# ZhangXiaze/DeepPointMap

Measured on AMD Instinct MI355X. Metric: LiDAR frames/s (encode+match+register), 65 536 pts/frame, higher is better.
Workload: dtype f32 (attention scores K Q^T and P V, Linear / Conv1d (+ LayerNorm) layers with K <= 2048 as exact three-way bf16 splits: 6 bf16 products per fp32 product, fp32 accumulate -- fp32 accuracy, bf16 matrix pipe; all else fp32); 1 GPU; synthetic 64x65536-pt scans per GPU: Encoder.forward + consecutive-frame registration_forward (256x256) + information matrix per frame; points_per_frame=65536, parallelism=frame-sharded x1, one RCCL gather of descriptors+edges per step, weights=procedural (deeppointmap_amd/weights.py), allocator_reserve_gib=16, geometry_waits_for_caller_stream=True

## Files before the change

### deeppointmap_amd/_lib.py

```python
from __future__ import annotations

import ctypes
import os

import torch
from ctypes import c_char_p, c_double, c_int, c_longlong, c_size_t, c_void_p

_HERE = os.path.dirname(os.path.abspath(__file__))
LIB_PATH = os.environ.get("DPM_LIB") or os.path.join(_HERE, "libdpm_hip.so")
VERSION_EXPERIMENT = 0x40000000

P, I, D, LL = c_void_p, c_int, c_double, c_longlong

SIGNATURES = {
    "dpm_version": (I, []),
    "dpm_error_string": (c_char_p, [I]),
    "dpm_prepare_points": (I, [P, P, I, I, I, P, P, P]),
    "dpm_to_channel_first": (I, [P, I, I, I, P, P]),
    "dpm_to_channel_first_ld": (I, [P, I, I, I, P, I, P]),
    "dpm_emit_descriptors": (I, [P, P, P, I, I, I, D, P, P, P, P, P]),
    "dpm_nested_levels": (I, [P, P, I, I, I, P, P, P, P, P]),
    "dpm_gather_frames": (I, [P, LL, I, I, I, P, I, P, P]),
    "dpm_fps_workspace_bytes": (c_size_t, [I, I, I]),
    "dpm_fps": (I, [P, P, I, I, I, P, P, P, P, P]),
    "dpm_fps_ex": (I, [P, P, I, I, I, P, P, P, P, I, P]),
    "dpm_fps_start": (I, [P, P, P, I, I, I, P, P, P, P, P]),
    "dpm_knn_workspace_bytes": (c_size_t, [I, I]),
    "dpm_knn_hybrid": (I, [P, P, P, I, I, I, I, D, P, P, P]),
    "dpm_knn_hybrid_reuse": (I, [P, P, P, I, I, I, I, D, P, P, P, P, P]),
    "dpm_knn_build_grid": (I, [P, P, I, I, D, P, P]),
    "dpm_knn_hybrid_prebuilt": (I, [P, P, P, I, I, I, I, D, P, P, P]),
    "dpm_ball_query": (I, [P, P, P, I, I, I, I, D, P, P]),
    "dpm_voxel_sampler_bounds": (I, [P, P, I, I, I, D, D, P, P]),
    "dpm_voxel_sampler_workspace_bytes": (c_size_t, [I, I, LL]),
    "dpm_voxel_sampler_select": (I, [P, P, I, I, I, D, D, P, LL, I, P, I, P, P, P]),
    "dpm_posegraph_optimize": (I, [P, I, P, P, P, P, I, I, P, P, P]),
    "dpm_host_topk_replay": (I, [P, I, I, I, P]),
    "dpm_host_sort_replay": (I, [P, I, I, P]),
    "dpm_group_mlp_max": (I, [P, P, P, P, P, P, P, P, I, I, I, I, I, I, D, P, P]),
    "dpm_group_mlp_max_generic": (I, [P, P, P, P, P, P, P, P, I, I, I, I, I, I, D, P, P]),
    "dpm_group_mlp_max_from_xyz": (I, [P, P, P, P, P, P, P, P, P, I, I, I, I, I, I, D, P, P]),
    "dpm_group_gather_ln_max": (I, [P, P, P, P, P, I, P, P, I, I, I, I, I, D, P, P]),
    "dpm_group_gather_ln_max_folded": (I, [P, P, P, P, I, P, P, I, I, I, I, I, D, P, P]),
    "dpm_group_affine_ln_max": (I, [P, P, P, P, P, P, I, P, P, I, I, I, I, I, D, P, P]),
    "dpm_group_gather_ln_max_centred": (I, [P, P, P, P, I, P, P, I, I, I, I, I, D, P, P]),
    "dpm_group_affine_ln_max_centred": (I, [P, P, P, P, P, P, I, P, P, I, I, I, I, I, D, P, P]),
    "dpm_linear": (I, [P, I, P, I, P, P, I, P, I, I, I, I, I, P]),
    "dpm_linear_batched": (I, [P, I, LL, P, I, LL, P, P, I, LL, P, I, LL, I, I, I, I, I, P]),
    "dpm_split_bf16x3": (I, [P, LL, P, P]),
    "dpm_linear_bf16x3": (I, [P, I, P, I, LL, P, P, I, P, I, I, I, I, I, P]),
    "dpm_linear_bf16x3_rank3": (I, [P, I, P, I, LL, P, P, I, P, I, I, I, I, I, P, P, I, D, P]),
    "dpm_linear_layernorm_bf16x3": (I, [P, I, P, I, LL, P, P, P, P, P, P, I, I, I, I, I, P]),
    "dpm_pwconv_pair_bf16x3": (I, [P, I, P, LL, P, P, P, P, LL, P, P, P, P, P, I, I, I, P]),
    "dpm_layernorm": (I, [P, I, P, P, P, P, P, I, I, I, I, P]),
    "dpm_linear_layernorm": (I, [P, I, P, I, P, P, P, P, P, P, I, I, I, I, I, P]),
    "dpm_three_interp_cat": (I, [P, P, P, P, P, I, I, I, I, I, P, P]),
    "dpm_posemb": (I, [P, I, P, I, I, I, P, P]),
    "dpm_attention": (I, [P, I, LL, P, I, LL, P, I, LL, P, I, LL, I, I, I, I, I, P]),
    "dpm_attention_shifted": (I, [P, I, LL, P, I, LL, P, I, LL, P, I, LL, I, I, I, I, I, I, P]),
    "dpm_attention_masked": (I, [P, I, LL, P, I, LL, P, I, LL, P, I, LL, I, I, I, I, I, I, P, P]),
    "dpm_attention_indexed": (I, [P, I, LL, P, I, LL, P, I, LL, P, I, LL, I, I, I, I, I, I, P, P]),
    "dpm_attention_split_workspace_bytes": (c_size_t, [I, I, I, I, I]),
# ... 56 lines not shown
    "dpm_offset_pairs_segment_sum": (I, [P, I, P, P, LL, I, P, P]),
    "dpm_group_train_forward": (I, [P, P, P, P, P, I, P, P, I, I, I, I, I, D, P, P, P]),
    "dpm_group_train_workspace_bytes": (c_size_t, [I, I, I, I, I]),
    "dpm_group_train_backward": (I, [P, P, P, P, P, I, P, I, I, I, I, I, D, P, P, P, P, P, P, P, P]),
    "dpm_loop_pool_workspace_bytes": (c_size_t, [I, I, I]),
    "dpm_loop_pool_forward": (I, [P, I, P, P, I, I, I, P, P, P]),
    "dpm_loop_pool_backward": (I, [P, I, P, P, P, I, I, I, P, P, P, P]),
    "dpm_loop_bce_forward": (I, [P, P, I, P, P, P, P]),
    "dpm_dense_train_workspace_bytes": (c_size_t, [LL, I, I]),
    "dpm_dense_train_forward": (I, [P, I, P, I, P, P, P, P, P, LL, I, I, I, P, P, P, P]),
    "dpm_dense_train_backward_rows": (I, [P, P, P, P, P, LL, I, I, P, P, P, P, P, P]),
    "dpm_dense_train_backward_gemm": (I, [P, P, I, P, I, LL, I, I, P, P, P, P, P]),
    "dpm_map_poses": (I, [P, P, P, P, P, I, I, I, P, P, P]),
    "dpm_map_assemble_fwd": (I, [P, P, P, P, P, I, I, I, I, I, D, P, P, P, P, P, P, P]),
    "dpm_map_assemble_bwd": (I, [P, P, I, I, I, I, I, P, P]),
    "dpm_optim_chunk": (I, []),
    "dpm_optim_step": (I, [I, P, P, I, D, D, D, D, D, D, D, D, I, I, P]),
    "dpm_flat_pack": (I, [P, P, I, P, LL, P]),
    "dpm_flat_unpack": (I, [P, P, I, P, LL, P]),
    "dpm_optim_step_synced": (I, [I, P, P, I, D, D, D, D, D, D, D, D, I, I, P, I, LL, D, P]),
    "dpm_lidar_cull": (I, [P, P, I, P, P, I, D, I, P, P, P, P]),
    "dpm_lidar_cast": (I, [P, P, P, I, I, P, I, I, D, D, P, P, P, P]),
    "dpm_lidar_cull_sweep": (I, [P, P, I, P, P, P, I, I, D, I, P, P, P, P, P]),
    "dpm_lidar_cast_sweep": (I, [P, P, P, I, I, P, I, I, P, I, D, D, P, P, P, P]),
    "dpm_lidar_emit": (I, [P, P, P, P, I, I, P, P, D, P, P, I, P, P, P, P, P, P]),
    "dpm_scene_distance": (I, [P, I, P, I, D, I, D, D, D, P, P, P]),
    "dpm_cloud_nn_workspace_bytes": (c_size_t, [I, I]),
    "dpm_cloud_nn": (I, [P, I, P, I, D, D, D, D, P, P, P, P]),
    "dpm_distance_stats_workspace_bytes": (c_size_t, [I, I, I]),
    "dpm_distance_stats": (I, [P, I, P, P, I, I, P, I, D, P, P, P]),
}


class DpmError(RuntimeError):
    pass


_lib = None


def load() -> ctypes.CDLL:
    global _lib
    if _lib is None:
        if not os.path.exists(LIB_PATH):
            raise DpmError(
                f"{LIB_PATH} not found: the HIP extension is not built. "
                "Run `python deeppointmap_amd/csrc/build.py` (there is no CPU fallback)."
            )
        lib = ctypes.CDLL(LIB_PATH)
        for name, (res, args) in SIGNATURES.items():
            fn = getattr(lib, name)
            fn.restype, fn.argtypes = res, args
        if lib.dpm_version() & VERSION_EXPERIMENT:
            import sys
            print(f"deeppointmap_amd: {LIB_PATH} is an EXPERIMENTAL build (-DDPM_EXPERIMENT): its kernels read DPM_* "
                  "measurement switches from the environment, some of which skip work -- not for results", file=sys.stderr)
        _lib = lib
    return _lib


def experimental() -> bool:
    return bool(load().dpm_version() & VERSION_EXPERIMENT)


def check(status: int, what: str) -> None:
    if status == 0:
# ... 6 lines not shown
```

### deeppointmap_amd/csrc/knn.hip

```cpp
#include "block_scan.h"
#include "filter_dc.h"
#include "topk_emulate.h"
#include <type_traits>

namespace {

constexpr int CPW = 4;
constexpr int WPB = 4;
constexpr int CAP = 512;
constexpr int KMAX = 64;
constexpr int TMPN = 128;
constexpr int GDIM = 128;
constexpr int GRID_MIN_N = 1024;
constexpr int KNN_TODO_MARK = -2;

using LdsF = __attribute__((address_space(3))) volatile float *;
using LdsI = __attribute__((address_space(3))) volatile int *;

__device__ __forceinline__ void wave_mem_sync() {
    __builtin_amdgcn_fence(__ATOMIC_SEQ_CST, "wavefront");
    __builtin_amdgcn_wave_barrier();
}

__device__ __forceinline__ float sq3(float x, float y, float z) { return (x * x + y * y) + z * z; }

__device__ __forceinline__ float exp_dist(float cx, float cy, float cz, float caa, float x, float y, float z,
                                          float bb) {
    return ((-2.f * fmaf(cz, z, fmaf(cy, y, cx * x))) + caa) + bb;
}

__device__ __forceinline__ int fkey(float d) {
    const int u = __float_as_int(d);
    return u >= 0 ? u : (u ^ 0x7fffffff);
}

// ... 276 lines not shown
    } else {
        for (int p = lane; p < c.cnt; p += 64) ti[p] = ci[p];
        wave_mem_sync();
    }
    const bool heap_regime = (long long)K * 64 <= (long long)N;
    bool exact_here = c.tie && len >= K && (heap_regime || tie_count || nth_row);
    if (exact_here && tie_count) {
        int slot = 0;
        if (lane == 0) slot = atomicAdd(tie_count, 1);
        slot = __shfl(slot, 0, 64);
        if (slot < TIE_CAP) {
            if (lane == 0) tie_rows[slot] = row;
            exact_here = false;
        }
    }
    if (exact_here && !heap_regime && !nth_row) exact_here = false;
    if (exact_here) {
        wave_mem_sync();
        if (heap_regime) heap_select_exact(pts, len, K, c.x, c.y, c.z, c.aa, cd, ci, td);
        else nth_select_exact(pts, len, N, K, c.x, c.y, c.z, c.aa, nth_row, cd, ci);
        emit_heap_result(cd, ci, K, r2, out);
    } else {
        int outv = (lane < k) ? ti[lane] : first;
        const unsigned long long hm = __ballot(lane < k && outv == first);
        const int L = hm ? __builtin_ctzll(hm) : 0;
        const int v0 = __shfl(outv, 0, 64);
        if (lane == L) outv = v0;
        if (lane == 0) outv = first;
        if (lane < K) out[lane] = outv;
    }
    wave_mem_sync();
}

__global__ __launch_bounds__(WPB * 64) void knn_hybrid_kernel(const float *__restrict__ points_all,
                                                              const int32_t *__restrict__ lengths,
                                                              const float *__restrict__ centers_all, int N,
                                                              int S, int K, float r2,
                                                              int32_t *__restrict__ idx_all,
                                                              const int32_t *__restrict__ reuse_idx,
                                                              const int32_t *__restrict__ center_src, int nth_rows) {
    extern __shared__ VI s_nth[];
    __shared__ float s_d[WPB][CPW][CAP];
    __shared__ int s_i[WPB][CPW][CAP];
    __shared__ float s_td[WPB][TMPN];
    __shared__ int s_ti[WPB][TMPN];
    const int b = blockIdx.y, w = threadIdx.x >> 6, lane = threadIdx.x & 63;
    const int s0 = (blockIdx.x * WPB + w) * CPW;
    if (s0 >= S) return;
    if (reuse_idx) {
        bool all = true;
        for (int j = 0; j < CPW && s0 + j < S; ++j) all &= center_src[(size_t)b * S + s0 + j] >= 0;
        if (all) {
            for (int j = 0; j < CPW && s0 + j < S; ++j) {
                const int src = center_src[(size_t)b * S + s0 + j];
                if (lane < K) idx_all[((size_t)b * S + s0 + j) * K + lane] = reuse_idx[((size_t)b * N + src) * K + lane];
            }
            return;
        }
    }
    const float *pts = points_all + (size_t)b * N * 3;
    const float *ctr = centers_all + (size_t)b * S * 3;
    const int len = min(max(lengths[b], 0), N);
    Ctr c[CPW];
#pragma unroll
    for (int j = 0; j < CPW; ++j) ctr_init(c[j], ctr + 3 * (size_t)min(s0 + j, S - 1), r2);
    for (int base = 0; base < len; base += 64) {
        const int i = base + lane;
        const bool ok = i < len;
        float x = 0.f, y = 0.f, z = 0.f;
        if (ok) x = pts[3 * i], y = pts[3 * i + 1], z = pts[3 * i + 2];
        const float bb = sq3(x, y, z);
#pragma unroll
        for (int j = 0; j < CPW; ++j) offer(c[j], ok, x, y, z, bb, i, K, (LdsF)s_d[w][j], (LdsI)s_i[w][j], (LdsF)s_td[w], (LdsI)s_ti[w]);
    }
#pragma unroll
    for (int j = 0; j < CPW; ++j) {
        if (s0 + j >= S) break;
        finish(c[j], pts, len, N, K, r2, (LdsF)s_d[w][j], (LdsI)s_i[w][j], (LdsF)s_td[w], (LdsI)s_ti[w],
               idx_all + ((size_t)b * S + (s0 + j)) * K, nullptr, nullptr, 0,
               nth_rows ? (VI *)((char *)s_nth + (size_t)w * N * (sizeof(VI) + 4)) : nullptr);
    }
}

struct KnnGrid {
    float lox, loy, inv_cs;
    int g;
    float err2;
    int H;
    int h;
    int pad;
};

constexpr float GRID_RHO_POINTS = 128.f;
constexpr float GRID_PI = 3.14159265f;

__global__ __launch_bounds__(1024) void knn_grid_build_kernel(const float *__restrict__ points_all,
                                                              const int32_t *__restrict__ lengths, int N,
                                                              float cs_min, float r2_margin, KnnGrid *__restrict__ hdr_all,
                                                              int *__restrict__ start_all,
                                                              float4 *__restrict__ sorted_all,
                                                              int *__restrict__ tie_count) {
    if (blockIdx.x == 0 && threadIdx.x == 0) tie_count[0] = 0, tie_count[1] = 0;
    __shared__ int s_hist[GDIM * GDIM];
    __shared__ float s_red[4][16];
    __shared__ float s_m2[16];
    __shared__ int s_wsum[16];
    const int b = blockIdx.x, t = threadIdx.x, lane = t & 63, w = t >> 6;
    const float *pts = points_all + (size_t)b * N * 3;
    const int len = min(max(lengths[b], 0), N);
    float lox = __builtin_inff(), loy = lox, hix = -lox, hiy = -lox, m2 = 0.f;
    constexpr int UB = 8;
    auto for_points = [&](auto &&fn) {
        for (int i0 = t; i0 < len; i0 += 1024 * UB) {
            float xs[UB], ys[UB], zs[UB];
// ... 881 lines not shown
}

extern "C" int dpm_knn_hybrid_reuse(const float *points, const int32_t *lengths, const float *centers, int B, int N,
                                    int S, int K, double radius, int32_t *idx, void *workspace,
                                    const int32_t *reuse_idx, const int32_t *center_src, dpm_stream_t stream) {
    DPM_CHECK_ARG(points && lengths && centers && idx);
    DPM_CHECK_ARG((reuse_idx == nullptr) == (center_src == nullptr));
    DPM_CHECK_ARG(B >= 1 && N >= 1 && S >= 1 && K >= 1 && radius > 0.0);
    if (K > KMAX) return DPM_EUNSUPPORTED;
    hipStream_t st = (hipStream_t)stream;
    const float r2 = (float)(radius * radius);
    if (N >= GRID_MIN_N && workspace) {
        const KnnWs w = carve(workspace, B, N);
        launch_grid_build(points, lengths, B, N, radius, w, st);
        return launch_grid_search(points, lengths, centers, B, N, S, K, r2, idx, w, reuse_idx, center_src, st);
    }
    int nth_rows = (long long)K * 64 > (long long)N;
    size_t dyn = nth_rows ? (sizeof(VI) + 4) * (size_t)WPB * N : 0;
    if (dyn) {
        static size_t static_lds = 0;
        if (!static_lds) {
            hipFuncAttributes fa;
            static_lds = hipFuncGetAttributes(&fa, (const void *)knn_hybrid_kernel) == hipSuccess ? fa.sharedSizeBytes : 72 * 1024;
        }
        if (static_lds + dyn > 160 * 1024) nth_rows = 0, dyn = 0;
        else if (dyn > 32 * 1024)
            (void)hipFuncSetAttribute((const void *)knn_hybrid_kernel, hipFuncAttributeMaxDynamicSharedMemorySize, (int)dyn);
    }
    hipLaunchKernelGGL(knn_hybrid_kernel, dim3(dpm_cdiv(S, WPB * CPW), B), dim3(WPB * 64), dyn, st, points, lengths, centers, N, S,
                       K, r2, idx, reuse_idx, center_src, nth_rows);
    return dpm_launch_status();
}

extern "C" int dpm_knn_build_grid(const float *points, const int32_t *lengths, int B, int N, double radius,
                                  void *workspace, dpm_stream_t stream) {
    DPM_CHECK_ARG(points && lengths && workspace && B >= 1 && N >= GRID_MIN_N && radius > 0.0);
    launch_grid_build(points, lengths, B, N, radius, carve(workspace, B, N), (hipStream_t)stream);
    return dpm_launch_status();
}

extern "C" int dpm_knn_hybrid_prebuilt(const float *points, const int32_t *lengths, const float *centers, int B, int N,
                                       int S, int K, double radius, int32_t *idx, void *workspace,
                                       dpm_stream_t stream) {
    DPM_CHECK_ARG(points && lengths && centers && idx && workspace);
    DPM_CHECK_ARG(B >= 1 && N >= GRID_MIN_N && S >= 1 && K >= 1 && radius > 0.0);
    if (K > KMAX) return DPM_EUNSUPPORTED;
    return launch_grid_search(points, lengths, centers, B, N, S, K, (float)(radius * radius), idx, carve(workspace, B, N),
                              nullptr, nullptr, (hipStream_t)stream);
}

extern "C" int dpm_knn_hybrid(const float *points, const int32_t *lengths, const float *centers, int B, int N,
                              int S, int K, double radius, int32_t *idx, void *workspace, dpm_stream_t stream) {
    return dpm_knn_hybrid_reuse(points, lengths, centers, B, N, S, K, radius, idx, workspace, nullptr, nullptr, stream);
}

extern "C" size_t dpm_knn_self_workspace_bytes(int N) { return dpm_knn_workspace_bytes(1, N > GRID_MIN_N ? N : GRID_MIN_N); }

extern "C" int dpm_knn_self(const float *xyz, int N, int K, double cell, int32_t *idx, float *dist2, float *mean_dist,
                            void *workspace, dpm_stream_t stream) {
    DPM_CHECK_ARG(xyz && workspace && N >= 1 && K >= 1 && cell > 0.0 && (idx || dist2 || mean_dist));
    if (K + 1 > KMAX) return DPM_EUNSUPPORTED;
    hipStream_t st = (hipStream_t)stream;
    uintptr_t p = ((uintptr_t)workspace + 255) & ~(uintptr_t)255;
    KnnGrid *hdr = (KnnGrid *)p;
    p = (p + sizeof(KnnGrid) + 255) & ~(uintptr_t)255;
    int *start = (int *)p;
// ... 119 lines not shown
```

### deeppointmap_amd/encoder.py

```python
from __future__ import annotations

from typing import List, Optional

import torch
from torch.utils.checkpoint import checkpoint

from . import ops
from .params import ParamTree, encoder_shapes


class Encoder(ParamTree):
    def __init__(self, args):
        super().__init__(encoder_shapes(args))
        self.args = args
        self.encoder_cfg = args.encoder
        self.in_channel = self.encoder_cfg.in_channel
        self.out_channel = self.encoder_cfg.out_channel
        self.downsample_layers = len(self.encoder_cfg.npoint)
        self.upsample_layers = self.encoder_cfg.upsample_layers
        for s in self.encoder_cfg.sample:
            if s["type"] not in ("fps", "fps-t3d", "voxel"):
                raise ValueError(f"{dict(s)} is not a supported sampling way, please use 'fps' or 'voxel'")
            if s["type"] == "voxel" and not ("size" in s and "range" in s):
                raise ValueError("a voxel sampler needs 'size' and 'range'")
        self.all_fps = all(s["type"] != "voxel" for s in self.encoder_cfg.sample)
        self.nested_fps = self.all_fps and all(b <= a for a, b in zip(self.encoder_cfg.npoint, self.encoder_cfg.npoint[1:]))
        self.presample_neighbours = False
        self.presample_neighbours_from = None
        self._price_tail = 0
        self.train_checkpoint_rows = 1 << 20
        self._was_trained = False
        self.eval()

    @property
    def device(self) -> torch.device:
        return self.p("point_mlp0.weight").device

    def _mlp_ln(self, x: torch.Tensor, conv: str, ln: str, act: int, post: Optional[torch.Tensor] = None):
        return ops.linear_layernorm(x, self.p(conv + ".weight"), self.p(conv + ".bias"), self.p(ln + ".weight"),
                                    self.p(ln + ".bias"), act=act, post=post)
# ... 60 lines not shown
                    if key not in answered and pts_i.shape[1] >= ops.GRID_MIN_N:
                        grids[("la", i, key)] = ops.knn_grid(pts_i, len_i, radii[j])
                    answered.add(key)
            out["grids"] = grids
            if n_levels == len(self.encoder_cfg.npoint):
                if self.presample_neighbours:
                    out["knn"] = self._neighbour_queries(out)
                elif self.presample_neighbours_from is not None:
                    out["knn"] = self._neighbour_queries(out, first_level=int(self.presample_neighbours_from))
        return out

    def _neighbour_queries(self, samp: dict, first_level: int = 0) -> dict:
        enc, grids, knn = self.encoder_cfg, samp.get("grids", {}), {}
        xyz, lengths, self_q = samp["xyz"], samp["lengths"], {}
        for i in range(len(enc.npoint)):
            radii, ks = enc.radius_list[i], enc.nsample_list[i]
            fidx, new_xyz, new_len = samp[f"fidx{i}"], samp[f"xyz{i}"], samp[f"len{i}"]
            if i < first_level:
                xyz, lengths, self_q = new_xyz, new_len, {}
                continue
            prev = self_q.get((float(radii[0]), int(ks[0])))
            knn[("sa", i)] = ops.knn_hybrid(xyz, lengths, new_xyz, ks[0], radii[0], reuse_idx=prev,
                                            center_src=fidx if prev is not None else None,
                                            grid=grids.get(("sa", i)) if prev is None else None)
            self_q = {}
            for j in range(1, len(radii)):
                key = (float(radii[j]), int(ks[j]))
                if key not in self_q:
                    self_q[key] = ops.knn_hybrid(new_xyz, new_len, new_xyz, ks[j], radii[j], grid=grids.get(("la", i, key)))
                knn[("la", i, key)] = self_q[key]
            xyz, lengths = new_xyz, new_len
        return knn

    @torch.no_grad()
    def forward(self, points: torch.Tensor, points_padding: torch.Tensor, trace: Optional[dict] = None,
                presampled: Optional[dict] = None, descriptor_scale: float = 0.0, spare_frames: int = 0,
                stop_level: Optional[int] = None, resume: Optional[dict] = None) -> List[torch.Tensor]:
        dev = self._require_gpu()
        if self.training and self.train_stage != "loop_detection":
            for name, given in (("presampled", presampled is not None), ("descriptor_scale", descriptor_scale != 0.0),
                                ("spare_frames", spare_frames != 0), ("stop_level", stop_level is not None),
                                ("resume", resume is not None)):
                if given:
                    raise ValueError(f"Encoder.forward: `{name}` belongs to the inference pipeline and is not available in "
                                     f".train() mode (call .eval() first)")
            return self._forward_train(points, points_padding, trace)
        enc = self.encoder_cfg
        if resume is not None:
            samp = resume["samp"]
        else:
            samp = presampled if presampled is not None else self.presample(points, points_padding)
        with torch.cuda.device(dev):
            pts, xyz, lengths = samp["pts"], samp["xyz"], samp["lengths"]
            w0 = self.p("point_mlp0.weight")
            fuse0 = (self.in_channel == 3 and w0.shape[0] % 4 == 0 and 2 * w0.shape[0] in (32, 64, 128)
                     and enc.nsample_list[0][0] in (16, 32))
            if resume is not None or fuse0:
                fea = None
            elif self.in_channel == 3:
                fea = ops.linear(xyz, w0, self.p("point_mlp0.bias"))
            else:
                fea = ops.linear(pts[:, :self.in_channel].transpose(1, 2).contiguous(), w0, self.p("point_mlp0.bias"))
            levels = [(xyz, fea, lengths)] if resume is None else resume["levels"]
            self_q = {} if resume is None else resume["self_q"]
            for i, npoint in enumerate(enc.npoint):
                if resume is not None and i < resume["next"]:
                    continue
                if stop_level is not None and i >= stop_level:
                    return dict(samp=samp, levels=levels, self_q=self_q, next=i)
                xyz, fea, lengths = levels[-1]
                radii, ks = enc.radius_list[i], enc.nsample_list[i]
                pre = f"downsampler.{i}"
                if f"fidx{i}" in samp:
                    fidx, new_xyz, new_len = samp[f"fidx{i}"], samp[f"xyz{i}"], samp[f"len{i}"]
                else:
                    fidx, new_xyz, new_len = self._sample_level(i, xyz, lengths)
                for _rep in range(1 + (self._price_tail if i >= 3 else 0)):
                    prev = self_q.get((float(radii[0]), int(ks[0])))
                    grids, knn = samp.get("grids", {}), samp.get("knn", {})
                    gidx = knn.get(("sa", i))
                    if gidx is None:
                        gidx = ops.knn_hybrid(xyz, lengths, new_xyz, ks[0], radii[0], reuse_idx=prev,
                                              center_src=fidx if prev is not None else None,
                                              grid=grids.get(("sa", i)) if prev is None else None)
                    self_q = {}
                    if fea is None:
                        m = pre + ".sa.mlp"
                        new_fea = ops.group_mlp_max_from_xyz(xyz, w0, self.p("point_mlp0.bias"), new_xyz, gidx,
                                                             self.p(m + ".0.weight"), self.p(m + ".0.bias"),
                                                             self.p(m + ".1.ln.weight"), self.p(m + ".1.ln.bias"), radii[0])
                    else:
                        new_fea = self._group(pre + ".sa.mlp", radii[0], xyz, fea, new_xyz, gidx)
                    if trace is not None:
                        trace[pre + ".fps.idx"], trace[pre + ".fps.new"] = fidx, new_xyz
                        trace[pre + ".sa.idx"], trace[pre + ".sa.out"] = gidx, new_fea
                    for j in range(1, len(radii)):
                        q = f"{pre}.irm.{j - 1}"
                        key = (float(radii[j]), int(ks[j]))
                        if key not in self_q:
                            self_q[key] = knn[("la", i, key)] if ("la", i, key) in knn else ops.knn_hybrid(
                                new_xyz, new_len, new_xyz, ks[j], radii[j], grid=grids.get(("la", i, key)))
                        lidx = self_q[key]
                        t = self._group(q + ".la.mlp", radii[j], new_xyz, new_fea, new_xyz, lidx)
                        pair = ops.pwconv_pair(t, self.p(q + ".pw_conv.0.weight"), self.p(q + ".pw_conv.0.bias"),
                                               self.p(q + ".pw_conv.1.ln.weight"), self.p(q + ".pw_conv.1.ln.bias"),
                                               self.p(q + ".pw_conv.3.weight"), self.p(q + ".pw_conv.3.bias"),
                                               self.p(q + ".pw_conv.4.ln.weight"), self.p(q + ".pw_conv.4.ln.bias"), post=new_fea)
                        if pair is not None:
                            new_fea = pair
                        else:
                            u = self._mlp_ln(t, q + ".pw_conv.0", q + ".pw_conv.1.ln", ops.ACT_RELU)
                            new_fea = self._mlp_ln(u, q + ".pw_conv.3", q + ".pw_conv.4.ln", ops.ACT_RELU, post=new_fea)
# ... 119 lines not shown
```

### deeppointmap_amd/knobs.py

```python
from __future__ import annotations

import os

FPS_ALGO = None
FUSED_LN = True
GEMM_BF16X3 = True
BF16X3_MAX_K = 2048
GEMM_LN_BF16X3 = True
BF16X3_LN_MIN_K = 128
FUSED_LN_SMALL_ROWS = 0
FOLD_GATHER = True
FOLD_MIN_RADIUS = 0.2
CENTRED_GATHER = True
FUSED_PWCONV = True
FUSED_MATCH = True
KV_PLANES = True
DEDUP_FRAMES = True

_ENV = {"DPM_FOLD_MIN_RADIUS": ("FOLD_MIN_RADIUS", float), "DPM_KV_PLANES": ("KV_PLANES", lambda v: v != "0"), "DPM_CENTRED_GATHER": ("CENTRED_GATHER", lambda v: v != "0"), "DPM_FPS_ALGO": ("FPS_ALGO", int), "DPM_NO_FUSED_LN": ("FUSED_LN", lambda v: v != "1"),
        "DPM_DEDUP_FRAMES": ("DEDUP_FRAMES", lambda v: v != "0"), "DPM_GEMM_BF16X3": ("GEMM_BF16X3", lambda v: v == "1"), "DPM_BF16X3_MAX_K": ("BF16X3_MAX_K", int), "DPM_BF16X3_LN_MIN_K": ("BF16X3_LN_MIN_K", int), "DPM_FUSED_LN_SMALL_ROWS": ("FUSED_LN_SMALL_ROWS", int), "DPM_GEMM_LN_BF16X3": ("GEMM_LN_BF16X3", lambda v: v == "1"),
        "DPM_FUSED_MATCH": ("FUSED_MATCH", lambda v: v != "0"), "DPM_FUSED_PWCONV": ("FUSED_PWCONV", lambda v: v != "0"), "DPM_FOLD_GATHER": ("FOLD_GATHER", lambda v: v != "0")}


def env_knobs() -> dict:
    return {k: v for k, v in sorted(os.environ.items()) if k.startswith("DPM_")}


def apply_env() -> dict:
    g = globals()
    for var, (name, conv) in _ENV.items():
        if var in os.environ:
            g[name] = conv(os.environ[var])
    return env_knobs()
```

### deeppointmap_amd/ops.py

```python
from __future__ import annotations

from typing import Optional, Tuple

import ctypes
import threading
import weakref

import torch

from . import _lib, knobs

ACT_NONE, ACT_RELU, ACT_SIGMOID = 0, 1, 2


def _ptr(t: Optional[torch.Tensor]):
    return None if t is None else t.data_ptr()


def _stream(t: torch.Tensor):
    return torch.cuda.current_stream(t.device).cuda_stream


def _chk(t: torch.Tensor, dtype, name: str):
    if not t.is_cuda:
# ... 112 lines not shown
    lib = _lib.load()
    ws = torch.empty(lib.dpm_knn_workspace_bytes(B, N), device=points.device, dtype=torch.uint8)
    _lib.check(lib.dpm_knn_build_grid(_ptr(points), _ptr(lengths), B, N, float(radius), _ptr(ws), _stream(points)),
               "dpm_knn_build_grid")
    return ws


def knn_hybrid(points: torch.Tensor, lengths: torch.Tensor, centers: torch.Tensor, K: int,
               radius: float, brute: bool = False, reuse_idx: Optional[torch.Tensor] = None,
               center_src: Optional[torch.Tensor] = None, grid: Optional[torch.Tensor] = None) -> torch.Tensor:
    _chk(points, torch.float32, "points")
    _chk(centers, torch.float32, "centers")
    _chk(lengths, torch.int32, "lengths")
    B, N, _ = points.shape
    S = centers.shape[1]
    idx = torch.empty(B, S, K, device=points.device, dtype=torch.int32)
    lib = _lib.load()
    if grid is not None:
        if brute or reuse_idx is not None or grid.numel() != lib.dpm_knn_workspace_bytes(B, N):
            raise ValueError("grid= goes with a plain grid search of the (B, N) it was built for")
        _lib.check(lib.dpm_knn_hybrid_prebuilt(_ptr(points), _ptr(lengths), _ptr(centers), B, N, S, K, float(radius),
                                               _ptr(idx), _ptr(grid), _stream(points)), "dpm_knn_hybrid_prebuilt")
        return idx
    nbytes = 0 if brute else lib.dpm_knn_workspace_bytes(B, N)
    ws = torch.empty(nbytes, device=points.device, dtype=torch.uint8) if nbytes else None
    if reuse_idx is not None:
        _chk(reuse_idx, torch.int32, "reuse_idx"), _chk(center_src, torch.int32, "center_src")
        if tuple(reuse_idx.shape) != (B, N, K) or tuple(center_src.shape) != (B, S):
            raise ValueError("reuse_idx must be (B,N,K) and center_src (B,S)")
    _lib.check(lib.dpm_knn_hybrid_reuse(_ptr(points), _ptr(lengths), _ptr(centers), B, N, S, K, float(radius),
                                        _ptr(idx), _ptr(ws), _ptr(reuse_idx), _ptr(center_src), _stream(points)),
               "dpm_knn_hybrid")
    return idx


def ball_query(points: torch.Tensor, lengths: torch.Tensor, centers: torch.Tensor, K: int, radius: float) -> torch.Tensor:
    _chk(points, torch.float32, "points"), _chk(centers, torch.float32, "centers"), _chk(lengths, torch.int32, "lengths")
    B, N, _ = points.shape
    S = centers.shape[1]
    idx = torch.empty(B, S, K, device=points.device, dtype=torch.int32)
    _lib.check(_lib.load().dpm_ball_query(_ptr(points), _ptr(lengths), _ptr(centers), B, N, S, K, float(radius),
                                          _ptr(idx), _stream(points)), "dpm_ball_query")
    return idx


VOXEL_SAMPLER_MAX_CELLS = 1 << 28
VOXEL_SAMPLER_MAX_WORKSPACE = 64 << 30


def voxel_sample(points: torch.Tensor, padding: torch.Tensor, K: Optional[int], voxel_size: float = 0.3,
                 sample_range: float = 1.0):
    _chk(points, torch.float32, "points")
    if padding.dtype != torch.bool or tuple(padding.shape) != tuple(points.shape[:2]):
        raise ValueError("points_padding must be a (B,N) bool tensor")
    B, N, D = points.shape
    if K is None and B != 1:
        raise ValueError("K=None takes one frame (utils.py:200)")
    lib, dev, st = _lib.load(), points.device, _stream(points)
    pad = padding.contiguous().view(torch.uint8)
    hdr = torch.empty(B, 8, device=dev, dtype=torch.float32)
    _lib.check(lib.dpm_voxel_sampler_bounds(_ptr(points), _ptr(pad), B, N, D, float(voxel_size), float(sample_range),
                                            _ptr(hdr), st), "dpm_voxel_sampler_bounds")
    dims = hdr[:, 3:6].double().cpu()
    if not bool(torch.isfinite(dims).all()):
        raise ValueError("voxel sampler: the frame's bounding box is not finite")
    cells = int(dims.prod(1).max().item())
# ... 1682 lines not shown
```

### include/dpm_hip.h

```cpp
#ifndef DPM_HIP_H
#define DPM_HIP_H

#include <stddef.h>
#include <stdint.h>

#ifdef __cplusplus
extern "C" {
#endif

typedef void *dpm_stream_t;

#define DPM_OK 0
#define DPM_EINVAL (-1)
#define DPM_EUNSUPPORTED (-2)

#define DPM_ACT_NONE 0
#define DPM_ACT_RELU 1
#define DPM_ACT_SIGMOID 2

#define DPM_VERSION_EXPERIMENT 0x40000000
int dpm_version(void);
const char *dpm_error_string(int status);

int dpm_prepare_points(const float *points_cf, const uint8_t *padding, int B, int C, int N,
                       float *xyz, int32_t *lengths, dpm_stream_t stream);

int dpm_to_channel_first(const float *x, int B, int R, int C, float *out, dpm_stream_t stream);
int dpm_to_channel_first_ld(const float *x, int B, int R, int C, float *out, int ldo, dpm_stream_t stream);

int dpm_emit_descriptors(const float *xyz, const float *fea, const int32_t *lengths, int B, int S, int C,
                         double coor_scale, float *coor, float *feat, uint8_t *padding, float *desc, dpm_stream_t stream);

int dpm_nested_levels(const float *xyz0, const int32_t *len0, int B, int K0, int n_levels, const int32_t *npoint,
                      float *xyz_out, int32_t *idx_out, int32_t *len_out, dpm_stream_t stream);

int dpm_gather_frames(const float *src, long long frame_stride, int rows, int ld, int cols, const int32_t *index, int n,
                      float *out, dpm_stream_t stream);

size_t dpm_fps_workspace_bytes(int B, int N, int K);
int dpm_fps(const float *xyz, const int32_t *lengths, int B, int N, int K, int32_t *idx,
            float *new_xyz, int32_t *new_lengths, void *workspace, dpm_stream_t stream);
int dpm_fps_ex(const float *xyz, const int32_t *lengths, int B, int N, int K, int32_t *idx,
               float *new_xyz, int32_t *new_lengths, void *workspace, int algo, dpm_stream_t stream);
int dpm_fps_start(const float *xyz, const int32_t *lengths, const int32_t *start, int B, int N, int K, int32_t *idx,
                  float *new_xyz, int32_t *new_lengths, void *workspace, dpm_stream_t stream);

size_t dpm_knn_workspace_bytes(int B, int N);
int dpm_knn_hybrid(const float *points, const int32_t *lengths, const float *centers, int B, int N,
                   int S, int K, double radius, int32_t *idx, void *workspace, dpm_stream_t stream);

int dpm_knn_hybrid_reuse(const float *points, const int32_t *lengths, const float *centers, int B, int N,
                         int S, int K, double radius, int32_t *idx, void *workspace, const int32_t *reuse_idx,
                         const int32_t *center_src, dpm_stream_t stream);

int dpm_knn_build_grid(const float *points, const int32_t *lengths, int B, int N, double radius, void *workspace,
                       dpm_stream_t stream);
int dpm_knn_hybrid_prebuilt(const float *points, const int32_t *lengths, const float *centers, int B, int N,
                            int S, int K, double radius, int32_t *idx, void *workspace, dpm_stream_t stream);

int dpm_ball_query(const float *points, const int32_t *lengths, const float *centers, int B, int N, int S,
                   int K, double radius, int32_t *idx, dpm_stream_t stream);

int dpm_voxel_sampler_bounds(const float *points, const uint8_t *padding, int B, int N, int D, double voxel_size,
                             double sample_range, float *hdr, dpm_stream_t stream);
size_t dpm_voxel_sampler_workspace_bytes(int B, int N, long long max_cells);
int dpm_voxel_sampler_select(const float *points, const uint8_t *padding, int B, int N, int D, double voxel_size,
                             double sample_range, float *hdr, long long max_cells, int K, int32_t *sel, int cap,
                             int32_t *n_unique, void *workspace, dpm_stream_t stream);


int dpm_posegraph_optimize(const double *poses, int n, const int32_t *src, const int32_t *dst, const double *X,
                           const double *info, int E, int reference_node, const double *criteria, double *out_poses,
                           double *stats);

int dpm_host_topk_replay(const float *values, int n, int k, int largest, int32_t *out_idx);
int dpm_host_sort_replay(const float *values, int n, int descending, int32_t *out_idx);

int dpm_group_mlp_max_generic(const float *xyz, const float *fea, const float *centers,
                              const int32_t *idx, const float *W, const float *bias, const float *gamma,
                              const float *beta, int B, int N, int S, int K, int Cin, int Cout, double radius,
                              float *out, dpm_stream_t stream);
int dpm_group_mlp_max(const float *xyz, const float *fea, const float *centers, const int32_t *idx,
                      const float *W, const float *bias, const float *gamma, const float *beta,
                      int B, int N, int S, int K, int Cin, int Cout, double radius, float *out,
                      dpm_stream_t stream);

// ... 317 lines not shown
```

Before: 16390 frames/s.

## Batch tail-level KNN queries into a single multi-query kernel launch

```diff
diff --git a/deeppointmap_amd/_lib.py b/deeppointmap_amd/_lib.py
--- a/deeppointmap_amd/_lib.py
+++ b/deeppointmap_amd/_lib.py
@@ -28,6 +28,7 @@
     "dpm_knn_workspace_bytes": (c_size_t, [I, I]),
     "dpm_knn_hybrid": (I, [P, P, P, I, I, I, I, D, P, P, P]),
     "dpm_knn_hybrid_reuse": (I, [P, P, P, I, I, I, I, D, P, P, P, P, P]),
+    "dpm_knn_hybrid_batch": (I, [P, I, I, P]),
     "dpm_knn_build_grid": (I, [P, P, I, I, D, P, P]),
     "dpm_knn_hybrid_prebuilt": (I, [P, P, P, I, I, I, I, D, P, P, P]),
     "dpm_ball_query": (I, [P, P, P, I, I, I, I, D, P, P]),
@@ -150,6 +151,11 @@
 }
 
 
+class KnnQuery(ctypes.Structure):
+    _fields_ = [("points", P), ("lengths", P), ("centers", P), ("idx", P), ("reuse_idx", P), ("center_src", P),
+                ("N", I), ("S", I), ("K", I), ("reserved", I), ("radius", D)]
+
+
 class DpmError(RuntimeError):
     pass
 
diff --git a/deeppointmap_amd/csrc/knn.hip b/deeppointmap_amd/csrc/knn.hip
--- a/deeppointmap_amd/csrc/knn.hip
+++ b/deeppointmap_amd/csrc/knn.hip
@@ -1,6 +1,7 @@
 #include "block_scan.h"
 #include "filter_dc.h"
 #include "topk_emulate.h"
+#include <algorithm>
 #include <type_traits>
 
 namespace {
@@ -343,6 +344,53 @@
     wave_mem_sync();
 }
 
+__device__ __forceinline__ void knn_hybrid_block(const float *__restrict__ points_all, const int32_t *__restrict__ lengths,
+                                                 const float *__restrict__ centers_all, int N, int S, int K, float r2,
+                                                 int32_t *__restrict__ idx_all, const int32_t *__restrict__ reuse_idx,
+                                                 const int32_t *__restrict__ center_src, int nth_rows, int bx, int wpb) {
+    extern __shared__ VI s_nth[];
+    __shared__ float s_d[WPB][CPW][CAP];
+    __shared__ int s_i[WPB][CPW][CAP];
+    __shared__ float s_td[WPB][TMPN];
+    __shared__ int s_ti[WPB][TMPN];
+    const int b = blockIdx.y, w = threadIdx.x >> 6, lane = threadIdx.x & 63;
+    const int s0 = (bx * wpb + w) * CPW;
+    if (w >= wpb || s0 >= S) return;
+    if (reuse_idx) {
+        bool all = true;
+        for (int j = 0; j < CPW && s0 + j < S; ++j) all &= center_src[(size_t)b * S + s0 + j] >= 0;
+        if (all) {
+            for (int j = 0; j < CPW && s0 + j < S; ++j) {
+                const int src = center_src[(size_t)b * S + s0 + j];
+                if (lane < K) idx_all[((size_t)b * S + s0 + j) * K + lane] = reuse_idx[((size_t)b * N + src) * K + lane];
+            }
+            return;
+        }
+    }
+    const float *pts = points_all + (size_t)b * N * 3;
+    const float *ctr = centers_all + (size_t)b * S * 3;
+    const int len = min(max(lengths[b], 0), N);
+    Ctr c[CPW];
+#pragma unroll
+    for (int j = 0; j < CPW; ++j) ctr_init(c[j], ctr + 3 * (size_t)min(s0 + j, S - 1), r2);
+    for (int base = 0; base < len; base += 64) {
+        const int i = base + lane;
+        const bool ok = i < len;
+        float x = 0.f, y = 0.f, z = 0.f;
+        if (ok) x = pts[3 * i], y = pts[3 * i + 1], z = pts[3 * i + 2];
+        const float bb = sq3(x, y, z);
+#pragma unroll
+        for (int j = 0; j < CPW; ++j) offer(c[j], ok, x, y, z, bb, i, K, (LdsF)s_d[w][j], (LdsI)s_i[w][j], (LdsF)s_td[w], (LdsI)s_ti[w]);
+    }
+#pragma unroll
+    for (int j = 0; j < CPW; ++j) {
+        if (s0 + j >= S) break;
+        finish(c[j], pts, len, N, K, r2, (LdsF)s_d[w][j], (LdsI)s_i[w][j], (LdsF)s_td[w], (LdsI)s_ti[w],
+               idx_all + ((size_t)b * S + (s0 + j)) * K, nullptr, nullptr, 0,
+               nth_rows ? (VI *)((char *)s_nth + (size_t)w * N * (sizeof(VI) + 4)) : nullptr);
+    }
+}
+
 __global__ __launch_bounds__(WPB * 64) void knn_hybrid_kernel(const float *__restrict__ points_all,
                                                               const int32_t *__restrict__ lengths,
                                                               const float *__restrict__ centers_all, int N,
@@ -350,47 +398,27 @@
                                                               int32_t *__restrict__ idx_all,
                                                               const int32_t *__restrict__ reuse_idx,
                                                               const int32_t *__restrict__ center_src, int nth_rows) {
-    extern __shared__ VI s_nth[];
-    __shared__ float s_d[WPB][CPW][CAP];
-    __shared__ int s_i[WPB][CPW][CAP];
-    __shared__ float s_td[WPB][TMPN];
-    __shared__ int s_ti[WPB][TMPN];
-    const int b = blockIdx.y, w = threadIdx.x >> 6, lane = threadIdx.x & 63;
-    const int s0 = (blockIdx.x * WPB + w) * CPW;
-    if (s0 >= S) return;
-    if (reuse_idx) {
-        bool all = true;
-        for (int j = 0; j < CPW && s0 + j < S; ++j) all &= center_src[(size_t)b * S + s0 + j] >= 0;
-        if (all) {
-            for (int j = 0; j < CPW && s0 + j < S; ++j) {
-                const int src = center_src[(size_t)b * S + s0 + j];
-                if (lane < K) idx_all[((size_t)b * S + s0 + j) * K + lane] = reuse_idx[((size_t)b * N + src) * K + lane];
-            }
-            return;
-        }
-    }
-    const float *pts = points_all + (size_t)b * N * 3;
-    const float *ctr = centers_all + (size_t)b * S * 3;
-    const int len = min(max(lengths[b], 0), N);
-    Ctr c[CPW];
-#pragma unroll
-    for (int j = 0; j < CPW; ++j) ctr_init(c[j], ctr + 3 * (size_t)min(s0 + j, S - 1), r2);
-    for (int base = 0; base < len; base += 64) {
-        const int i = base + lane;
-        const bool ok = i < len;
-        float x = 0.f, y = 0.f, z = 0.f;
-        if (ok) x = pts[3 * i], y = pts[3 * i + 1], z = pts[3 * i + 2];
-        const float bb = sq3(x, y, z);
-#pragma unroll
-        for (int j = 0; j < CPW; ++j) offer(c[j], ok, x, y, z, bb, i, K, (LdsF)s_d[w][j], (LdsI)s_i[w][j], (LdsF)s_td[w], (LdsI)s_ti[w]);
-    }
-#pragma unroll
-    for (int j = 0; j < CPW; ++j) {
-        if (s0 + j >= S) break;
-        finish(c[j], pts, len, N, K, r2, (LdsF)s_d[w][j], (LdsI)s_i[w][j], (LdsF)s_td[w], (LdsI)s_ti[w],
-               idx_all + ((size_t)b * S + (s0 + j)) * K, nullptr, nullptr, 0,
-               nth_rows ? (VI *)((char *)s_nth + (size_t)w * N * (sizeof(VI) + 4)) : nullptr);
-    }
+    knn_hybrid_block(points_all, lengths, centers_all, N, S, K, r2, idx_all, reuse_idx, center_src, nth_rows, blockIdx.x, WPB);
+}
+
+constexpr int KNN_BATCH_MAX = 8;
+struct KnnBatch {
+    int n;
+    int first[KNN_BATCH_MAX + 1];
+    struct {
+        const float *points, *centers;
+        const int32_t *lengths, *reuse_idx, *center_src;
+        int32_t *idx;
+        int N, S, K, nth_rows, wpb;
+        float r2;
+    } q[KNN_BATCH_MAX];
+};
+
+__global__ __launch_bounds__(WPB * 64) void knn_hybrid_batch_kernel(KnnBatch kb) {
+    int j = 0;
+    while (j + 1 < kb.n && (int)blockIdx.x >= kb.first[j + 1]) ++j;
+    knn_hybrid_block(kb.q[j].points, kb.q[j].lengths, kb.q[j].centers, kb.q[j].N, kb.q[j].S, kb.q[j].K, kb.q[j].r2, kb.q[j].idx,
+                     kb.q[j].reuse_idx, kb.q[j].center_src, kb.q[j].nth_rows, (int)blockIdx.x - kb.first[j], kb.q[j].wpb);
 }
 
 struct KnnGrid {
@@ -1338,6 +1366,41 @@
     return dpm_launch_status();
 }
 
+extern "C" int dpm_knn_hybrid_batch(const dpm_knn_query *queries, int n_queries, int B, dpm_stream_t stream) {
+    DPM_CHECK_ARG(queries && n_queries >= 1 && n_queries <= KNN_BATCH_MAX && B >= 1);
+    KnnBatch kb;
+    kb.n = n_queries;
+    long long blocks = 0;
+    size_t dyn = 0;
+    for (int j = 0; j < n_queries; ++j)
+        if (!queries[j].reuse_idx && (long long)queries[j].K * 64 > (long long)queries[j].N && queries[j].N >= 1)
+            dyn = std::max(dyn, (sizeof(VI) + 4) * (size_t)WPB * queries[j].N);
+    const size_t dyn_plain = dyn;
+    for (int j = 0; j < n_queries; ++j) {
+        const dpm_knn_query &q = queries[j];
+        DPM_CHECK_ARG(q.points && q.lengths && q.centers && q.idx);
+        DPM_CHECK_ARG((q.reuse_idx == nullptr) == (q.center_src == nullptr));
+        DPM_CHECK_ARG(q.N >= 1 && q.N < GRID_MIN_N && q.S >= 1 && q.K >= 1 && q.radius > 0.0);
+        if (q.K > KMAX) return DPM_EUNSUPPORTED;
+        const int nth_rows = (long long)q.K * 64 > (long long)q.N;
+        const size_t d = nth_rows ? (sizeof(VI) + 4) * (size_t)WPB * q.N : 0;
+        const int wpb = q.reuse_idx && d > dyn_plain ? 1 : WPB;
+        dyn = std::max(dyn, d / WPB * wpb);
+        kb.first[j] = (int)blocks;
+        kb.q[j].points = q.points, kb.q[j].centers = q.centers, kb.q[j].lengths = q.lengths;
+        kb.q[j].reuse_idx = q.reuse_idx, kb.q[j].center_src = q.center_src, kb.q[j].idx = q.idx;
+        kb.q[j].N = q.N, kb.q[j].S = q.S, kb.q[j].K = q.K, kb.q[j].nth_rows = nth_rows, kb.q[j].wpb = wpb;
+        kb.q[j].r2 = (float)(q.radius * q.radius);
+        blocks += dpm_cdiv(q.S, wpb * CPW);
+    }
+    kb.first[n_queries] = (int)blocks;
+    if (blocks > 0x7fffffffLL) return DPM_EUNSUPPORTED;
+    if (dyn > 32 * 1024)
+        (void)hipFuncSetAttribute((const void *)knn_hybrid_batch_kernel, hipFuncAttributeMaxDynamicSharedMemorySize, (int)dyn);
+    hipLaunchKernelGGL(knn_hybrid_batch_kernel, dim3((unsigned)blocks, B), dim3(WPB * 64), dyn, (hipStream_t)stream, kb);
+    return dpm_launch_status();
+}
+
 extern "C" int dpm_knn_build_grid(const float *points, const int32_t *lengths, int B, int N, double radius,
                                   void *workspace, dpm_stream_t stream) {
     DPM_CHECK_ARG(points && lengths && workspace && B >= 1 && N >= GRID_MIN_N && radius > 0.0);
diff --git a/deeppointmap_amd/encoder.py b/deeppointmap_amd/encoder.py
--- a/deeppointmap_amd/encoder.py
+++ b/deeppointmap_amd/encoder.py
@@ -5,7 +5,7 @@
 import torch
 from torch.utils.checkpoint import checkpoint
 
-from . import ops
+from . import knobs, ops
 from .params import ParamTree, encoder_shapes
 
 
@@ -132,6 +132,35 @@
             xyz, lengths = new_xyz, new_len
         return knn
 
+    def _tail_first_level(self) -> int:
+        enc = self.encoder_cfg
+        L = len(enc.npoint)
+        first = L - 2
+        if first < 1 or max(enc.npoint[first - 1:L - 1]) >= ops.GRID_MIN_N:
+            return L
+        la_first = {(float(r), int(k)) for r, k in zip(enc.radius_list[first][1:], enc.nsample_list[first][1:])}
+        if (float(enc.radius_list[L - 1][0]), int(enc.nsample_list[L - 1][0])) in la_first:
+            return L
+        n = sum(1 + len({(float(r), int(k)) for r, k in zip(enc.radius_list[i][1:], enc.nsample_list[i][1:])}) for i in (first, L - 1))
+        return first if n <= 8 else L
+
+    def _tail_neighbour_queries(self, samp: dict, first: int, xyz, lengths, self_q: dict) -> dict:
+        enc, queries, keys = self.encoder_cfg, [], []
+        for i in range(first, len(enc.npoint)):
+            radii, ks = enc.radius_list[i], enc.nsample_list[i]
+            fidx, new_xyz, new_len = samp[f"fidx{i}"], samp[f"xyz{i}"], samp[f"len{i}"]
+            prev = self_q.get((float(radii[0]), int(ks[0]))) if i == first else None
+            queries.append(dict(points=xyz, lengths=lengths, centers=new_xyz, K=ks[0], radius=radii[0], reuse_idx=prev,
+                                center_src=fidx if prev is not None else None))
+            keys.append(("sa", i))
+            for j in range(1, len(radii)):
+                key = ("la", i, (float(radii[j]), int(ks[j])))
+                if key not in keys:
+                    queries.append(dict(points=new_xyz, lengths=new_len, centers=new_xyz, K=ks[j], radius=radii[j]))
+                    keys.append(key)
+            xyz, lengths = new_xyz, new_len
+        return dict(zip(keys, ops.knn_hybrid_batch(queries)))
+
     @torch.no_grad()
     def forward(self, points: torch.Tensor, points_padding: torch.Tensor, trace: Optional[dict] = None,
                 presampled: Optional[dict] = None, descriptor_scale: float = 0.0, spare_frames: int = 0,
@@ -163,6 +192,7 @@
                 fea = ops.linear(pts[:, :self.in_channel].transpose(1, 2).contiguous(), w0, self.p("point_mlp0.bias"))
             levels = [(xyz, fea, lengths)] if resume is None else resume["levels"]
             self_q = {} if resume is None else resume["self_q"]
+            tail_first, tail_knn = (self._tail_first_level() if knobs.FUSED_TAIL else len(enc.npoint)), {}
             for i, npoint in enumerate(enc.npoint):
                 if resume is not None and i < resume["next"]:
                     continue
@@ -178,6 +208,9 @@
                 for _rep in range(1 + (self._price_tail if i >= 3 else 0)):
                     prev = self_q.get((float(radii[0]), int(ks[0])))
                     grids, knn = samp.get("grids", {}), samp.get("knn", {})
+                    if i == tail_first and ("sa", i) not in knn and all(f"fidx{j}" in samp for j in range(i, len(enc.npoint))):
+                        tail_knn = self._tail_neighbour_queries(samp, i, xyz, lengths, self_q)
+                    knn = {**tail_knn, **knn} if i >= tail_first else knn
                     gidx = knn.get(("sa", i))
                     if gidx is None:
                         gidx = ops.knn_hybrid(xyz, lengths, new_xyz, ks[0], radii[0], reuse_idx=prev,
diff --git a/deeppointmap_amd/knobs.py b/deeppointmap_amd/knobs.py
--- a/deeppointmap_amd/knobs.py
+++ b/deeppointmap_amd/knobs.py
@@ -15,11 +15,13 @@
 FUSED_PWCONV = True
 FUSED_MATCH = True
 KV_PLANES = True
+FUSED_TAIL = True
 DEDUP_FRAMES = True
 
 _ENV = {"DPM_FOLD_MIN_RADIUS": ("FOLD_MIN_RADIUS", float), "DPM_KV_PLANES": ("KV_PLANES", lambda v: v != "0"), "DPM_CENTRED_GATHER": ("CENTRED_GATHER", lambda v: v != "0"), "DPM_FPS_ALGO": ("FPS_ALGO", int), "DPM_NO_FUSED_LN": ("FUSED_LN", lambda v: v != "1"),
         "DPM_DEDUP_FRAMES": ("DEDUP_FRAMES", lambda v: v != "0"), "DPM_GEMM_BF16X3": ("GEMM_BF16X3", lambda v: v == "1"), "DPM_BF16X3_MAX_K": ("BF16X3_MAX_K", int), "DPM_BF16X3_LN_MIN_K": ("BF16X3_LN_MIN_K", int), "DPM_FUSED_LN_SMALL_ROWS": ("FUSED_LN_SMALL_ROWS", int), "DPM_GEMM_LN_BF16X3": ("GEMM_LN_BF16X3", lambda v: v == "1"),
-        "DPM_FUSED_MATCH": ("FUSED_MATCH", lambda v: v != "0"), "DPM_FUSED_PWCONV": ("FUSED_PWCONV", lambda v: v != "0"), "DPM_FOLD_GATHER": ("FOLD_GATHER", lambda v: v != "0")}
+        "DPM_FUSED_MATCH": ("FUSED_MATCH", lambda v: v != "0"), "DPM_FUSED_PWCONV": ("FUSED_PWCONV", lambda v: v != "0"), "DPM_FOLD_GATHER": ("FOLD_GATHER", lambda v: v != "0"),
+        "DPM_FUSED_TAIL": ("FUSED_TAIL", lambda v: v != "0")}
 
 
 def env_knobs() -> dict:
diff --git a/deeppointmap_amd/ops.py b/deeppointmap_amd/ops.py
--- a/deeppointmap_amd/ops.py
+++ b/deeppointmap_amd/ops.py
@@ -168,6 +168,31 @@
                                         _ptr(idx), _ptr(ws), _ptr(reuse_idx), _ptr(center_src), _stream(points)),
                "dpm_knn_hybrid")
     return idx
+
+
+def knn_hybrid_batch(queries) -> list:
+    arr = (_lib.KnnQuery * len(queries))()
+    out, B = [], queries[0]["points"].shape[0]
+    for a, q in zip(arr, queries):
+        points, lengths, centers = q["points"], q["lengths"], q["centers"]
+        reuse_idx, center_src, K = q.get("reuse_idx"), q.get("center_src"), int(q["K"])
+        _chk(points, torch.float32, "points"), _chk(centers, torch.float32, "centers"), _chk(lengths, torch.int32, "lengths")
+        N, S = points.shape[1], centers.shape[1]
+        if points.shape[0] != B or centers.shape[0] != B or lengths.shape[0] != B or N >= GRID_MIN_N:
+            raise ValueError(f"knn_hybrid_batch: every query takes the same {B} frames of fewer than {GRID_MIN_N} points")
+        if (reuse_idx is None) != (center_src is None):
+            raise ValueError("reuse_idx and center_src go together")
+        if reuse_idx is not None:
+            _chk(reuse_idx, torch.int32, "reuse_idx"), _chk(center_src, torch.int32, "center_src")
+            if tuple(reuse_idx.shape) != (B, N, K) or tuple(center_src.shape) != (B, S):
+                raise ValueError("reuse_idx must be (B,N,K) and center_src (B,S)")
+        idx = torch.empty(B, S, K, device=points.device, dtype=torch.int32)
+        a.points, a.lengths, a.centers, a.idx = _ptr(points), _ptr(lengths), _ptr(centers), _ptr(idx)
+        a.reuse_idx, a.center_src, a.N, a.S, a.K, a.radius = _ptr(reuse_idx), _ptr(center_src), N, S, K, float(q["radius"])
+        out.append(idx)
+    _lib.check(_lib.load().dpm_knn_hybrid_batch(ctypes.cast(arr, ctypes.c_void_p), len(queries), B,
+                                                _stream(queries[0]["points"])), "dpm_knn_hybrid_batch")
+    return out
 
 
 def ball_query(points: torch.Tensor, lengths: torch.Tensor, centers: torch.Tensor, K: int, radius: float) -> torch.Tensor:
diff --git a/include/dpm_hip.h b/include/dpm_hip.h
--- a/include/dpm_hip.h
+++ b/include/dpm_hip.h
@@ -52,6 +52,18 @@
 int dpm_knn_hybrid_reuse(const float *points, const int32_t *lengths, const float *centers, int B, int N,
                          int S, int K, double radius, int32_t *idx, void *workspace, const int32_t *reuse_idx,
                          const int32_t *center_src, dpm_stream_t stream);
+
+typedef struct dpm_knn_query {
+    const float *points;
+    const int32_t *lengths;
+    const float *centers;
+    int32_t *idx;
+    const int32_t *reuse_idx;
+    const int32_t *center_src;
+    int N, S, K, reserved;
+    double radius;
+} dpm_knn_query;
+int dpm_knn_hybrid_batch(const dpm_knn_query *queries, int n_queries, int B, dpm_stream_t stream);
 
 int dpm_knn_build_grid(const float *points, const int32_t *lengths, int B, int N, double radius, void *workspace,
                        dpm_stream_t stream);
```

Result: slower. 16140 frames/s (-1.5%).
